# filaPro/unidet3d

Hardware: AMD Instinct MI355X
Metric: scenes/sec fwd+bwd, 100k-pt ScanNet voxel grid, 1/2/4/8 MI355X (higher is better)
Workload: dtype f32

## Files before the change

### unidet3d_amd/csrc/bn.hip

```cpp
#include <stdlib.h>

#include "u3d_common.h"

namespace u3d {

struct BnFin {
    double* sums;
    double rows;
    int set_rows;
    const float* gamma;
    const float* beta;
    float eps, momentum;
    float* running_mean;
    float* running_var;
    float* st;
    int64_t* nbt;
};

__device__ __forceinline__ void bn_finalize_channel(double s1, double s2, double rows, const float* gamma, const float* beta, float eps,
                                                    float momentum, float* running_mean, float* running_var, float* mean, float* invstd,
                                                    float* scale, float* shift, int c) {
#pragma clang fp contract(off)
    const double m = s1 / rows;
    double var = fma(-m, m, s2 / rows);
    if (var < 0.0) var = 0.0;
    const float is = (float)(1.0 / sqrt(var + (double)eps));
    const float mf = (float)m;
    mean[c] = mf;
    invstd[c] = is;
    const float sc = gamma[c] * is;
    scale[c] = sc;
    shift[c] = fmaf(-mf, sc, beta[c]);
    if (running_mean) {
        const double unbiased = rows > 1.0 ? var * rows / (rows - 1.0) : var;
        const float keep = 1.f - momentum;
        const float km = keep * running_mean[c], kv = keep * running_var[c];
        const float nm = momentum * mf, nv = momentum * (float)unbiased;
        running_mean[c] = km + nm;
        running_var[c] = kv + nv;
    }
}

__device__ __forceinline__ void bn_finish_body(const double* partial, int nblk, int C, const BnFin& f, int wave0, int nw, bool first) {
    const int lane = threadIdx.x & 63;
    for (int c = wave0; c < C; c += nw) {
        double t1 = 0.0, t2 = 0.0;
        for (int b = lane; b < nblk; b += 64) {
            t1 += partial[(int64_t)b * 2 * C + c];
            t2 += partial[(int64_t)b * 2 * C + C + c];
        }
#pragma unroll
        for (int d = 32; d >= 1; d >>= 1) { t1 += __shfl_xor(t1, d, 64); t2 += __shfl_xor(t2, d, 64); }
        if (lane) continue;
        f.sums[c] = t1;
        f.sums[C + c] = t2;
        if (!f.st) continue;
        bn_finalize_channel(t1, t2, f.rows, f.gamma, f.beta, f.eps, f.momentum, f.running_mean, f.running_var, f.st, f.st + C,
                            f.st + 2 * C, f.st + 3 * C, c);
    }
    if (first && threadIdx.x == 0) {
        if (f.set_rows) f.sums[2 * C] = f.rows;
        if (f.nbt) *f.nbt += 1;
    }
}

__global__ __launch_bounds__(256) void bn_sum_k(const double* __restrict__ partial, int nblk, int C, BnFin f) {
    bn_finish_body(partial, nblk, C, f, blockIdx.x * 4 + (threadIdx.x >> 6), gridDim.x * 4, blockIdx.x == 0);
}

template <int MODE>
__global__ __launch_bounds__(256) void bn_reduce_k(const float* __restrict__ x, const float* __restrict__ dy,
                                                   const float* __restrict__ mean, const float* __restrict__ invstd,
                                                   const float* __restrict__ scale, const float* __restrict__ shift, int relu,
                                                   int64_t n, int C, double* sums ) {
    __shared__ double sh[256 * 8];
    const int lpr = C >> 2;
    const int rpb = 256 / lpr;
    const int tid = threadIdx.x;
    const int c4 = tid % lpr, slot = tid / lpr;
    double a[4] = {0, 0, 0, 0}, b[4] = {0, 0, 0, 0};
    if (slot < rpb) {
        float4 mu = make_float4(0, 0, 0, 0), is = mu, sc = mu, sf = mu;
        if (MODE == 1) {
            mu = *reinterpret_cast<const float4*>(mean + c4 * 4);
            is = *reinterpret_cast<const float4*>(invstd + c4 * 4);
            sc = *reinterpret_cast<const float4*>(scale + c4 * 4);
            sf = *reinterpret_cast<const float4*>(shift + c4 * 4);
        }
        const int64_t stride = (int64_t)gridDim.x * rpb;
        for (int64_t r0 = (int64_t)blockIdx.x * rpb + slot; r0 < n; r0 += 4 * stride) {
            float4 v4[4], g4[4];
#pragma unroll
            for (int u = 0; u < 4; ++u) {
                const int64_t r = r0 + u * stride;
                v4[u] = make_float4(0.f, 0.f, 0.f, 0.f);
                g4[u] = make_float4(0.f, 0.f, 0.f, 0.f);
                if (r < n) {
                    v4[u] = *reinterpret_cast<const float4*>(x + r * C + c4 * 4);
                    if (MODE == 1) g4[u] = *reinterpret_cast<const float4*>(dy + r * C + c4 * 4);
                }
            }
#pragma unroll
            for (int u = 0; u < 4; ++u) {
                const float4 v = v4[u];
                if (MODE == 0) {
                    a[0] += v.x; a[1] += v.y; a[2] += v.z; a[3] += v.w;
                    b[0] += (double)v.x * v.x; b[1] += (double)v.y * v.y; b[2] += (double)v.z * v.z; b[3] += (double)v.w * v.w;
                } else {
                    float4 g = g4[u];
                    if (relu) {
                        if (!(v.x * sc.x + sf.x > 0.f)) g.x = 0.f;
                        if (!(v.y * sc.y + sf.y > 0.f)) g.y = 0.f;
                        if (!(v.z * sc.z + sf.z > 0.f)) g.z = 0.f;
                        if (!(v.w * sc.w + sf.w > 0.f)) g.w = 0.f;
                    }
                    a[0] += g.x; a[1] += g.y; a[2] += g.z; a[3] += g.w;
                    b[0] += (double)g.x * ((v.x - mu.x) * is.x); b[1] += (double)g.y * ((v.y - mu.y) * is.y);
                    b[2] += (double)g.z * ((v.z - mu.z) * is.z); b[3] += (double)g.w * ((v.w - mu.w) * is.w);
                }
            }
        }
    }
#pragma unroll
    for (int j = 0; j < 4; ++j) { sh[tid * 8 + j] = a[j]; sh[tid * 8 + 4 + j] = b[j]; }
    __syncthreads();
    if (tid < lpr) {
        double ta[4] = {0, 0, 0, 0}, tb[4] = {0, 0, 0, 0};
        for (int s = 0; s < rpb; ++s) {
            const int o = (s * lpr + tid) * 8;
#pragma unroll
            for (int j = 0; j < 4; ++j) { ta[j] += sh[o + j]; tb[j] += sh[o + 4 + j]; }
        }
        double* out = sums + (int64_t)blockIdx.x * 2 * C;
#pragma unroll
        for (int j = 0; j < 4; ++j) {
            out[tid * 4 + j] = ta[j];
            out[C + tid * 4 + j] = tb[j];
        }
    }
}

__global__ __launch_bounds__(256) void bn_partials_k(const float* __restrict__ partial, int64_t n_tiles, int C, double* ws) {
    __shared__ double sh[256];
    const int C2 = 2 * C, tid = threadIdx.x;
    double* out = ws + (int64_t)blockIdx.x * C2;
    for (int c0 = 0; c0 < C2; c0 += 256) {
        const int w = min(256, C2 - c0), rpp = 256 / w;
        const int col = c0 + tid % w, slot = tid / w;
        double a0 = 0.0, a1 = 0.0;
        if (slot < rpp) {
            const int64_t step = (int64_t)gridDim.x * rpp;
            int64_t r = (int64_t)blockIdx.x * rpp + slot;
            for (; r + step < n_tiles; r += 2 * step) {
                a0 += (double)partial[r * C2 + col];
                a1 += (double)partial[(r + step) * C2 + col];
            }
            if (r < n_tiles) a0 += (double)partial[r * C2 + col];
        }
        sh[tid] = a0 + a1;
        __syncthreads();
        if (tid < w) {
            double t = 0.0;
            for (int s_ = 0; s_ < rpp; ++s_) t += sh[s_ * w + tid];
            out[c0 + tid] = t;
        }
        __syncthreads();
    }
}


__global__ void bn_finalize_k(const double* __restrict__ sums, double count, const float* __restrict__ gamma,
                              const float* __restrict__ beta, float eps, float momentum, float* running_mean,
                              float* running_var, int C, float* mean, float* invstd, float* scale, float* shift,
                              int64_t* num_batches_tracked) {
    const int c = blockIdx.x * blockDim.x + threadIdx.x;
    if (c == 0 && num_batches_tracked) *num_batches_tracked += 1;
    if (c >= C) return;
    if (!(count > 0.0)) count = sums[2 * C];
    bn_finalize_channel(sums[c], sums[C + c], count, gamma, beta, eps, momentum, running_mean, running_var, mean, invstd, scale, shift, c);
}


__global__ __launch_bounds__(256) void bn_apply_k(const float* __restrict__ x, const float* __restrict__ scale,
                                                  const float* __restrict__ shift, int relu, int64_t n4, int C4, float* y, __bf16* yb) {
    for (int64_t i = (int64_t)blockIdx.x * blockDim.x + threadIdx.x; i < n4; i += (int64_t)gridDim.x * blockDim.x) {
        const int c4 = (int)(i % C4);
        const float4 v = reinterpret_cast<const float4*>(x)[i];
        const float4 sc = reinterpret_cast<const float4*>(scale)[c4];
        const float4 sf = reinterpret_cast<const float4*>(shift)[c4];
        const float4 o = bn_affine_relu(v, sc, sf, relu);
        reinterpret_cast<float4*>(y)[i] = o;
        if (yb) store_shadow(yb, i / C4, C4, 0, c4, o);
    }
}

__global__ __launch_bounds__(256) void bn_bwd_apply_k(const float* __restrict__ x, const float* __restrict__ dy,
                                                      const float* __restrict__ mean, const float* __restrict__ invstd,
                                                      const float* __restrict__ scale, const float* __restrict__ shift, int relu,
                                                      const double* __restrict__ sums, double inv_count, int64_t n4, int C,
                                                      float* dx, float* dgamma, float* dbeta, const double* __restrict__ count_src,
                                                      const float* __restrict__ addend, __bf16* dxb) {
    const int C4 = C >> 2;
    if (!(inv_count > 0.0)) inv_count = 1.0 / (count_src ? count_src[0] : sums[2 * C]);
    if (blockIdx.x == 0 && dgamma) {
        for (int c = threadIdx.x; c < C; c += blockDim.x) {
            dbeta[c] = (float)sums[c];
            dgamma[c] = (float)sums[C + c];
        }
    }
    for (int64_t i = (int64_t)blockIdx.x * blockDim.x + threadIdx.x; i < n4; i += (int64_t)gridDim.x * blockDim.x) {
        const int c4 = (int)(i % C4);
        const float4 v = reinterpret_cast<const float4*>(x)[i];
        float4 g = reinterpret_cast<const float4*>(dy)[i];
        const float4 mu = reinterpret_cast<const float4*>(mean)[c4];
        const float4 is = reinterpret_cast<const float4*>(invstd)[c4];
        const float4 sc = reinterpret_cast<const float4*>(scale)[c4];
        const float4 sf = reinterpret_cast<const float4*>(shift)[c4];
        if (relu) {
            if (!(v.x * sc.x + sf.x > 0.f)) g.x = 0.f;
            if (!(v.y * sc.y + sf.y > 0.f)) g.y = 0.f;
            if (!(v.z * sc.z + sf.z > 0.f)) g.z = 0.f;
            if (!(v.w * sc.w + sf.w > 0.f)) g.w = 0.f;
        }
        const int c = c4 * 4;
        const float m1x = (float)(sums[c] * inv_count), m1y = (float)(sums[c + 1] * inv_count);
        const float m1z = (float)(sums[c + 2] * inv_count), m1w = (float)(sums[c + 3] * inv_count);
        const float m2x = (float)(sums[C + c] * inv_count), m2y = (float)(sums[C + c + 1] * inv_count);
        const float m2z = (float)(sums[C + c + 2] * inv_count), m2w = (float)(sums[C + c + 3] * inv_count);
        float4 o;
        o.x = sc.x * (g.x - m1x - (v.x - mu.x) * is.x * m2x);
        o.y = sc.y * (g.y - m1y - (v.y - mu.y) * is.y * m2y);
        o.z = sc.z * (g.z - m1z - (v.z - mu.z) * is.z * m2z);
        o.w = sc.w * (g.w - m1w - (v.w - mu.w) * is.w * m2w);
        if (addend) {
            const float4 e = reinterpret_cast<const float4*>(addend)[i];
            o.x += e.x; o.y += e.y; o.z += e.z; o.w += e.w;
        }
        reinterpret_cast<float4*>(dx)[i] = o;
        if (dxb) store_shadow(dxb, i / C4, C4, 0, c4, o);
    }
}

static bool bn_ok(int64_t n, int C) { return n > 0 && C >= 4 && C <= 512 && C % 4 == 0; }
static bool shadow_ok(const void* sh, int C) { return !sh || C % 32 == 0; }
static unsigned ew_grid(int64_t n4) {
    int64_t g = ceil_div(n4, 256);
    return (unsigned)(g < 1 ? 1 : (g > 4096 ? 4096 : g));
}

}

using namespace u3d;

extern "C" {

static int bn_grid(int64_t n, int C) {
    const int rpb = 256 / (C / 4);
    int64_t g = ceil_div(n, (int64_t)rpb * 16);
    return (int)(g < 1 ? 1 : (g > 256 ? 256 : g));
}
static int bn_partials_grid(int64_t n_tiles, int C) {
    const int rpp = 2 * C >= 256 ? 1 : 256 / (2 * C);
    int64_t g = ceil_div(n_tiles, (int64_t)rpp * 16);
    return (int)(g < 1 ? 1 : (g > 128 ? 128 : g));
}

int64_t u3d_bn_ws_bytes(int C) { return (int64_t)256 * 2 * C * sizeof(double) + 64; }

static int bn_finish_launch(const void* ws, int nblk, int C, const BnFin& f, hipStream_t s) {
    hipLaunchKernelGGL(bn_sum_k, dim3((C + 3) / 4), dim3(256), 0, s, (const double*)ws, nblk, C, f);
    return check_launch("bn_sum");
}

static BnFin bn_fin(double* sums, double rows, int set_rows) {
    BnFin f;
    f.sums = sums; f.rows = rows; f.set_rows = set_rows; f.gamma = nullptr; f.beta = nullptr; f.eps = 0.f; f.momentum = 0.f;
    f.running_mean = nullptr; f.running_var = nullptr; f.st = nullptr; f.nbt = nullptr;
    return f;
}

static int bn_stats_launch(const float* x, int64_t n, int C, const float* partial, int64_t n_tiles, const BnFin& f, void* ws, hipStream_t s) {
    if (partial) {
        if (n_tiles <= 0) return U3D_EINVAL;
        ProfScope prof(U3D_K_BN, s, (double)n_tiles * C * 8);
        const int g = bn_partials_grid(n_tiles, C);
        hipLaunchKernelGGL(bn_partials_k, dim3(g), dim3(256), 0, s, partial, n_tiles, C, (double*)ws);
        return bn_finish_launch(ws, g, C, f, s);
    }
    ProfScope prof(U3D_K_BN, s, (double)n * C * 4);
    const int g = bn_grid(n, C);
    hipLaunchKernelGGL(bn_reduce_k<0>, dim3(g), dim3(256), 0, s, x, (const float*)nullptr, (const float*)nullptr,
                       (const float*)nullptr, (const float*)nullptr, (const float*)nullptr, 0, n, C, (double*)ws);
    return bn_finish_launch(ws, g, C, f, s);
}

int u3d_bn_stats(const float* x, int64_t n, int C, const float* partial, int64_t n_tiles, double* sums, void* ws, u3d_stream_t stream) {
    if ((!x && !partial) || !sums || !ws || !bn_ok(n, C)) return U3D_EINVAL;
    return bn_stats_launch(x, n, C, partial, n_tiles, bn_fin(sums, (double)n, 1), ws, (hipStream_t)stream);
}

int u3d_bn_finalize(const double* sums, double count, const float* gamma, const float* beta, float eps, float momentum,
                    float* running_mean, float* running_var, int C, float* mean, float* invstd, float* scale,
                    float* shift, int64_t* num_batches_tracked, u3d_stream_t stream) {
    if (!sums || !gamma || !beta || !mean || !invstd || !scale || !shift || C <= 0) return U3D_EINVAL;
    hipLaunchKernelGGL(bn_finalize_k, dim3((C + 63) / 64), dim3(64), 0, (hipStream_t)stream, sums, count, gamma, beta, eps,
                       momentum, running_mean, running_var, C, mean, invstd, scale, shift, num_batches_tracked);
    return check_launch("bn_finalize");
}

int u3d_bn_apply(const float* x, const float* scale, const float* shift, int relu, int64_t n, int C, float* y, void* y_bf16,
                 u3d_stream_t stream) {
    if (!x || !scale || !shift || !y || !bn_ok(n, C) || !shadow_ok(y_bf16, C)) return U3D_EINVAL;
    hipStream_t s = (hipStream_t)stream;
    ProfScope prof(U3D_K_BN, s, (double)n * C * (y_bf16 ? 10 : 8));
    const int64_t n4 = n * (C / 4);
    hipLaunchKernelGGL(bn_apply_k, dim3(ew_grid(n4)), dim3(256), 0, s, x, scale, shift, relu, n4, C / 4, y, (__bf16*)y_bf16);
    return check_launch("bn_apply");
}

int u3d_bn_bwd_stats(const float* x, const float* dy, const float* mean, const float* invstd, const float* scale,
                     const float* shift, int relu, int64_t n, int C, double* sums, void* ws, u3d_stream_t stream) {
    if (!x || !dy || !mean || !invstd || !scale || !shift || !sums || !ws || !bn_ok(n, C)) return U3D_EINVAL;
    hipStream_t s = (hipStream_t)stream;
    ProfScope prof(U3D_K_BN, s, (double)n * C * 8);
    const int g = bn_grid(n, C);
    const BnFin f = bn_fin(sums, 0.0, 0);
    hipLaunchKernelGGL(bn_reduce_k<1>, dim3(g), dim3(256), 0, s, x, dy, mean, invstd, scale, shift, relu, n, C, (double*)ws);
    return bn_finish_launch(ws, g, C, f, s);
}

int u3d_bn_bwd_apply(const float* x, const float* dy, const float* mean, const float* invstd, const float* scale,
                     const float* shift, int relu, const double* sums, double count, int64_t n, int C, float* dx, void* dx_bf16,
                     float* dgamma, float* dbeta, const float* addend, u3d_stream_t stream) {
    if (!x || !dy || !mean || !invstd || !scale || !shift || !sums || !dx || !bn_ok(n, C) || !shadow_ok(dx_bf16, C)) return U3D_EINVAL;
    hipStream_t s = (hipStream_t)stream;
    ProfScope prof(U3D_K_BN, s, (double)n * C * 12);
    const int64_t n4 = n * (C / 4);
    hipLaunchKernelGGL(bn_bwd_apply_k, dim3(ew_grid(n4)), dim3(256), 0, s, x, dy, mean, invstd, scale, shift, relu, sums,
                       1.0 / count, n4, C, dx, dgamma, dbeta, (const double*)nullptr, addend, (__bf16*)dx_bf16);
    return check_launch("bn_bwd_apply");
}

int u3d_bn_forward(const float* x, int64_t n, int C, const float* partial, int64_t n_tiles, const float* gamma, const float* beta, float eps,
                   float momentum, float* running_mean, float* running_var, int64_t* num_batches_tracked, int relu, float* y, void* y_bf16,
                   float* st, double* sums, void* ws, u3d_stream_t stream) {
    if (!x || !sums || !ws || !gamma || !beta || !st || !y || !bn_ok(n, C) || !shadow_ok(y_bf16, C)) return U3D_EINVAL;
    if (partial && n_tiles <= 0) return U3D_EINVAL;
    BnFin f = bn_fin(sums, (double)n, 1);
    f.gamma = gamma; f.beta = beta; f.eps = eps; f.momentum = momentum; f.running_mean = running_mean; f.running_var = running_var;
    f.st = st; f.nbt = num_batches_tracked;
    int rc = bn_stats_launch(x, n, C, partial, n_tiles, f, ws, (hipStream_t)stream);
    if (rc) return rc;
    return u3d_bn_apply(x, st + 2 * C, st + 3 * C, relu, n, C, y, y_bf16, stream);
}

int u3d_bn_backward(const float* x, const float* dy, const float* st, int relu, const double* fwd_sums, double* sums, int64_t n, int C,
                    float* dx, void* dx_bf16, float* dgamma, float* dbeta, const float* addend, void* ws, u3d_stream_t stream) {
    if (!fwd_sums || !st || !dx || !shadow_ok(dx_bf16, C)) return U3D_EINVAL;
    int rc = u3d_bn_bwd_stats(x, dy, st, st + C, st + 2 * C, st + 3 * C, relu, n, C, sums, ws, stream);
    if (rc) return rc;
    hipStream_t s = (hipStream_t)stream;
    ProfScope prof(U3D_K_BN, s, (double)n * C * 12);
    const int64_t n4 = n * (C / 4);
    hipLaunchKernelGGL(bn_bwd_apply_k, dim3(ew_grid(n4)), dim3(256), 0, s, x, dy, (const float*)st, (const float*)(st + C), (const float*)(st + 2 * C),
                       (const float*)(st + 3 * C), relu, (const double*)sums, -1.0, n4, C, dx, dgamma, dbeta, fwd_sums + 2 * C, addend,
                       (__bf16*)dx_bf16);
    return check_launch("bn_backward");
}

}
```

Measured before the change: 310.9.

## Add single-kernel slab BatchNorm paths for small inputs and hoist per-channel constants

```diff
diff --git a/unidet3d_amd/csrc/bn.hip b/unidet3d_amd/csrc/bn.hip
--- a/unidet3d_amd/csrc/bn.hip
+++ b/unidet3d_amd/csrc/bn.hip
@@ -68,7 +68,7 @@
     bn_finish_body(partial, nblk, C, f, blockIdx.x * 4 + (threadIdx.x >> 6), gridDim.x * 4, blockIdx.x == 0);
 }
 
-template <int MODE>
+template <int MODE, int TRIP>
 __global__ __launch_bounds__(256) void bn_reduce_k(const float* __restrict__ x, const float* __restrict__ dy,
                                                    const float* __restrict__ mean, const float* __restrict__ invstd,
                                                    const float* __restrict__ scale, const float* __restrict__ shift, int relu,
@@ -88,10 +88,10 @@
             sf = *reinterpret_cast<const float4*>(shift + c4 * 4);
         }
         const int64_t stride = (int64_t)gridDim.x * rpb;
-        for (int64_t r0 = (int64_t)blockIdx.x * rpb + slot; r0 < n; r0 += 4 * stride) {
-            float4 v4[4], g4[4];
-#pragma unroll
-            for (int u = 0; u < 4; ++u) {
+        for (int64_t r0 = (int64_t)blockIdx.x * rpb + slot; r0 < n; r0 += TRIP * stride) {
+            float4 v4[TRIP], g4[TRIP];
+#pragma unroll
+            for (int u = 0; u < TRIP; ++u) {
                 const int64_t r = r0 + u * stride;
                 v4[u] = make_float4(0.f, 0.f, 0.f, 0.f);
                 g4[u] = make_float4(0.f, 0.f, 0.f, 0.f);
@@ -101,7 +101,7 @@
                 }
             }
 #pragma unroll
-            for (int u = 0; u < 4; ++u) {
+            for (int u = 0; u < TRIP; ++u) {
                 const float4 v = v4[u];
                 if (MODE == 0) {
                     a[0] += v.x; a[1] += v.y; a[2] += v.z; a[3] += v.w;
@@ -183,15 +183,36 @@
 
 __global__ __launch_bounds__(256) void bn_apply_k(const float* __restrict__ x, const float* __restrict__ scale,
                                                   const float* __restrict__ shift, int relu, int64_t n4, int C4, float* y, __bf16* yb) {
-    for (int64_t i = (int64_t)blockIdx.x * blockDim.x + threadIdx.x; i < n4; i += (int64_t)gridDim.x * blockDim.x) {
-        const int c4 = (int)(i % C4);
+    const int64_t i0 = (int64_t)blockIdx.x * blockDim.x + threadIdx.x;
+    const int c4 = (int)(i0 % C4);
+    const float4 sc = reinterpret_cast<const float4*>(scale)[c4];
+    const float4 sf = reinterpret_cast<const float4*>(shift)[c4];
+    for (int64_t i = i0; i < n4; i += (int64_t)gridDim.x * blockDim.x) {
         const float4 v = reinterpret_cast<const float4*>(x)[i];
-        const float4 sc = reinterpret_cast<const float4*>(scale)[c4];
-        const float4 sf = reinterpret_cast<const float4*>(shift)[c4];
         const float4 o = bn_affine_relu(v, sc, sf, relu);
         reinterpret_cast<float4*>(y)[i] = o;
         if (yb) store_shadow(yb, i / C4, C4, 0, c4, o);
     }
+}
+
+struct BnBwdConst { float4 mu, is, sc, sf, m1, m2; };
+__device__ __forceinline__ float4 bn_bwd_elem(const float4& v, float4 g, const BnBwdConst& k, int relu, const float4* addend) {
+    if (relu) {
+        if (!(v.x * k.sc.x + k.sf.x > 0.f)) g.x = 0.f;
+        if (!(v.y * k.sc.y + k.sf.y > 0.f)) g.y = 0.f;
+        if (!(v.z * k.sc.z + k.sf.z > 0.f)) g.z = 0.f;
+        if (!(v.w * k.sc.w + k.sf.w > 0.f)) g.w = 0.f;
+    }
+    float4 o;
+    o.x = k.sc.x * (g.x - k.m1.x - (v.x - k.mu.x) * k.is.x * k.m2.x);
+    o.y = k.sc.y * (g.y - k.m1.y - (v.y - k.mu.y) * k.is.y * k.m2.y);
+    o.z = k.sc.z * (g.z - k.m1.z - (v.z - k.mu.z) * k.is.z * k.m2.z);
+    o.w = k.sc.w * (g.w - k.m1.w - (v.w - k.mu.w) * k.is.w * k.m2.w);
+    if (addend) {
+        const float4 e = *addend;
+        o.x += e.x; o.y += e.y; o.z += e.z; o.w += e.w;
+    }
+    return o;
 }
 
 __global__ __launch_bounds__(256) void bn_bwd_apply_k(const float* __restrict__ x, const float* __restrict__ dy,
@@ -208,44 +229,226 @@
             dgamma[c] = (float)sums[C + c];
         }
     }
-    for (int64_t i = (int64_t)blockIdx.x * blockDim.x + threadIdx.x; i < n4; i += (int64_t)gridDim.x * blockDim.x) {
-        const int c4 = (int)(i % C4);
+    const int64_t i0 = (int64_t)blockIdx.x * blockDim.x + threadIdx.x;
+    const int c4 = (int)(i0 % C4);
+    const int c = c4 * 4;
+    BnBwdConst k;
+    k.mu = reinterpret_cast<const float4*>(mean)[c4];
+    k.is = reinterpret_cast<const float4*>(invstd)[c4];
+    k.sc = reinterpret_cast<const float4*>(scale)[c4];
+    k.sf = reinterpret_cast<const float4*>(shift)[c4];
+    k.m1 = make_float4((float)(sums[c] * inv_count), (float)(sums[c + 1] * inv_count), (float)(sums[c + 2] * inv_count), (float)(sums[c + 3] * inv_count));
+    k.m2 = make_float4((float)(sums[C + c] * inv_count), (float)(sums[C + c + 1] * inv_count), (float)(sums[C + c + 2] * inv_count),
+                       (float)(sums[C + c + 3] * inv_count));
+    for (int64_t i = i0; i < n4; i += (int64_t)gridDim.x * blockDim.x) {
         const float4 v = reinterpret_cast<const float4*>(x)[i];
-        float4 g = reinterpret_cast<const float4*>(dy)[i];
-        const float4 mu = reinterpret_cast<const float4*>(mean)[c4];
-        const float4 is = reinterpret_cast<const float4*>(invstd)[c4];
-        const float4 sc = reinterpret_cast<const float4*>(scale)[c4];
-        const float4 sf = reinterpret_cast<const float4*>(shift)[c4];
-        if (relu) {
-            if (!(v.x * sc.x + sf.x > 0.f)) g.x = 0.f;
-            if (!(v.y * sc.y + sf.y > 0.f)) g.y = 0.f;
-            if (!(v.z * sc.z + sf.z > 0.f)) g.z = 0.f;
-            if (!(v.w * sc.w + sf.w > 0.f)) g.w = 0.f;
-        }
-        const int c = c4 * 4;
-        const float m1x = (float)(sums[c] * inv_count), m1y = (float)(sums[c + 1] * inv_count);
-        const float m1z = (float)(sums[c + 2] * inv_count), m1w = (float)(sums[c + 3] * inv_count);
-        const float m2x = (float)(sums[C + c] * inv_count), m2y = (float)(sums[C + c + 1] * inv_count);
-        const float m2z = (float)(sums[C + c + 2] * inv_count), m2w = (float)(sums[C + c + 3] * inv_count);
-        float4 o;
-        o.x = sc.x * (g.x - m1x - (v.x - mu.x) * is.x * m2x);
-        o.y = sc.y * (g.y - m1y - (v.y - mu.y) * is.y * m2y);
-        o.z = sc.z * (g.z - m1z - (v.z - mu.z) * is.z * m2z);
-        o.w = sc.w * (g.w - m1w - (v.w - mu.w) * is.w * m2w);
-        if (addend) {
-            const float4 e = reinterpret_cast<const float4*>(addend)[i];
-            o.x += e.x; o.y += e.y; o.z += e.z; o.w += e.w;
-        }
+        const float4 g = reinterpret_cast<const float4*>(dy)[i];
+        const float4 o = bn_bwd_elem(v, g, k, relu, addend ? reinterpret_cast<const float4*>(addend) + i : nullptr);
         reinterpret_cast<float4*>(dx)[i] = o;
         if (dxb) store_shadow(dxb, i / C4, C4, 0, c4, o);
     }
 }
 
+#define BN_SLAB_THREADS 1024
+#define BN_SLAB_WAVES (BN_SLAB_THREADS / 64)
+
+__device__ __forceinline__ void bn_slab_sum(const double* a, const double* b, double* sh) {
+    const int tid = threadIdx.x;
+    double v[8];
+#pragma unroll
+    for (int j = 0; j < 4; ++j) { v[j] = a[j]; v[4 + j] = b[j]; }
+#pragma unroll
+    for (int j = 0; j < 8; ++j) {
+#pragma unroll
+        for (int d = 32; d >= 1; d >>= 1) v[j] += __shfl_xor(v[j], d, 64);
+    }
+    if ((tid & 63) == 0) {
+#pragma unroll
+        for (int j = 0; j < 8; ++j) sh[(tid >> 6) * 8 + j] = v[j];
+    }
+    __syncthreads();
+    if (tid < 8) {
+        double t = 0.0;
+        for (int w = 0; w < BN_SLAB_WAVES; ++w) t += sh[w * 8 + tid];
+        sh[8 * BN_SLAB_WAVES + tid] = t;
+    }
+    __syncthreads();
+}
+
+__global__ __launch_bounds__(BN_SLAB_THREADS) void bn_slab_fwd_k(const float* __restrict__ x, int64_t n, int C, BnFin f, int relu, float* y, __bf16* yb) {
+    __shared__ double sh[8 * BN_SLAB_WAVES + 8];
+    __shared__ float cst[8];
+    const int C4 = C >> 2, c4 = blockIdx.x, tid = threadIdx.x;
+    const float4* xc = reinterpret_cast<const float4*>(x) + c4;
+    double a[4] = {0, 0, 0, 0}, b[4] = {0, 0, 0, 0};
+    for (int64_t r0 = tid; r0 < n; r0 += 4 * BN_SLAB_THREADS) {
+        float4 v4[4];
+#pragma unroll
+        for (int u = 0; u < 4; ++u) {
+            const int64_t r = r0 + u * BN_SLAB_THREADS;
+            v4[u] = r < n ? xc[r * C4] : make_float4(0.f, 0.f, 0.f, 0.f);
+        }
+#pragma unroll
+        for (int u = 0; u < 4; ++u) {
+            const float4 v = v4[u];
+            a[0] += v.x; a[1] += v.y; a[2] += v.z; a[3] += v.w;
+            b[0] += (double)v.x * v.x; b[1] += (double)v.y * v.y; b[2] += (double)v.z * v.z; b[3] += (double)v.w * v.w;
+        }
+    }
+    bn_slab_sum(a, b, sh);
+    if (tid < 4) {
+        const int c = c4 * 4 + tid;
+        const double t1 = sh[8 * BN_SLAB_WAVES + tid], t2 = sh[8 * BN_SLAB_WAVES + 4 + tid];
+        f.sums[c] = t1;
+        f.sums[C + c] = t2;
+        if (f.st) {
+            bn_finalize_channel(t1, t2, f.rows, f.gamma, f.beta, f.eps, f.momentum, f.running_mean, f.running_var, f.st, f.st + C, f.st + 2 * C,
+                                f.st + 3 * C, c);
+            cst[tid] = f.st[2 * C + c];
+            cst[4 + tid] = f.st[3 * C + c];
+        }
+    }
+    if (c4 == 0 && tid == 0) {
+        if (f.set_rows) f.sums[2 * C] = f.rows;
+        if (f.nbt) *f.nbt += 1;
+    }
+    if (!y) return;
+    __syncthreads();
+    const float4 sc = make_float4(cst[0], cst[1], cst[2], cst[3]), sf = make_float4(cst[4], cst[5], cst[6], cst[7]);
+    for (int64_t r = tid; r < n; r += BN_SLAB_THREADS) {
+        const float4 v = xc[r * C4];
+        const float4 o = bn_affine_relu(v, sc, sf, relu);
+        reinterpret_cast<float4*>(y)[r * C4 + c4] = o;
+        if (yb) store_shadow(yb, r, C4, 0, c4, o);
+    }
+}
+
+__global__ __launch_bounds__(BN_SLAB_THREADS) void bn_slab_bwd_k(const float* __restrict__ x, const float* __restrict__ dy,
+                                                                 const float* __restrict__ mean, const float* __restrict__ invstd,
+                                                                 const float* __restrict__ scale, const float* __restrict__ shift, int relu,
+                                                                 int64_t n, int C, double* sums, const double* __restrict__ count_src, float* dx,
+                                                                 float* dgamma, float* dbeta, const float* __restrict__ addend, __bf16* dxb) {
+    __shared__ double sh[8 * BN_SLAB_WAVES + 8];
+    const int C4 = C >> 2, c4 = blockIdx.x, tid = threadIdx.x;
+    const float4* xc = reinterpret_cast<const float4*>(x) + c4;
+    const float4* gc = reinterpret_cast<const float4*>(dy) + c4;
+    BnBwdConst k;
+    k.mu = reinterpret_cast<const float4*>(mean)[c4];
+    k.is = reinterpret_cast<const float4*>(invstd)[c4];
+    k.sc = reinterpret_cast<const float4*>(scale)[c4];
+    k.sf = reinterpret_cast<const float4*>(shift)[c4];
+    const float4 mu = k.mu, is = k.is, sc = k.sc, sf = k.sf;
+    double a[4] = {0, 0, 0, 0}, b[4] = {0, 0, 0, 0};
+    for (int64_t r0 = tid; r0 < n; r0 += 4 * BN_SLAB_THREADS) {
+        float4 v4[4], g4[4];
+#pragma unroll
+        for (int u = 0; u < 4; ++u) {
+            const int64_t r = r0 + u * BN_SLAB_THREADS;
+            v4[u] = make_float4(0.f, 0.f, 0.f, 0.f);
+            g4[u] = make_float4(0.f, 0.f, 0.f, 0.f);
+            if (r < n) { v4[u] = xc[r * C4]; g4[u] = gc[r * C4]; }
+        }
+#pragma unroll
+        for (int u = 0; u < 4; ++u) {
+            const float4 v = v4[u];
+            float4 g = g4[u];
+            if (relu) {
+                if (!(v.x * sc.x + sf.x > 0.f)) g.x = 0.f;
+                if (!(v.y * sc.y + sf.y > 0.f)) g.y = 0.f;
+                if (!(v.z * sc.z + sf.z > 0.f)) g.z = 0.f;
+                if (!(v.w * sc.w + sf.w > 0.f)) g.w = 0.f;
+            }
+            a[0] += g.x; a[1] += g.y; a[2] += g.z; a[3] += g.w;
+            b[0] += (double)g.x * ((v.x - mu.x) * is.x); b[1] += (double)g.y * ((v.y - mu.y) * is.y);
+            b[2] += (double)g.z * ((v.z - mu.z) * is.z); b[3] += (double)g.w * ((v.w - mu.w) * is.w);
+        }
+    }
+    bn_slab_sum(a, b, sh);
+    const double* tot = sh + 8 * BN_SLAB_WAVES;
+    if (tid < 4) {
+        const int c = c4 * 4 + tid;
+        sums[c] = tot[tid];
+        sums[C + c] = tot[4 + tid];
+        if (dx && dgamma) {
+            dbeta[c] = (float)tot[tid];
+            dgamma[c] = (float)tot[4 + tid];
+        }
+    }
+    if (!dx) return;
+    const double inv_count = 1.0 / count_src[0];
+    k.m1 = make_float4((float)(tot[0] * inv_count), (float)(tot[1] * inv_count), (float)(tot[2] * inv_count), (float)(tot[3] * inv_count));
+    k.m2 = make_float4((float)(tot[4] * inv_count), (float)(tot[5] * inv_count), (float)(tot[6] * inv_count), (float)(tot[7] * inv_count));
+    for (int64_t r = tid; r < n; r += BN_SLAB_THREADS) {
+        const int64_t i = r * C4 + c4;
+        const float4 o = bn_bwd_elem(xc[r * C4], gc[r * C4], k, relu, addend ? reinterpret_cast<const float4*>(addend) + i : nullptr);
+        reinterpret_cast<float4*>(dx)[i] = o;
+        if (dxb) store_shadow(dxb, r, C4, 0, c4, o);
+    }
+}
+
 static bool bn_ok(int64_t n, int C) { return n > 0 && C >= 4 && C <= 512 && C % 4 == 0; }
 static bool shadow_ok(const void* sh, int C) { return !sh || C % 32 == 0; }
-static unsigned ew_grid(int64_t n4) {
+static unsigned apply_grid(int64_t n4, int C4) {
     int64_t g = ceil_div(n4, 256);
-    return (unsigned)(g < 1 ? 1 : (g > 4096 ? 4096 : g));
+    g = g < 1 ? 1 : (g > 4096 ? 4096 : g);
+    int a = C4, b = 256;
+    while (b) { const int t = a % b; a = b; b = t; }
+    const int m = C4 / a;
+    return (unsigned)(ceil_div(g, m) * m);
+}
+
+#if defined(U3D_BN_CAP) && U3D_BN_CAP > 512
+#define BN_MAX_GRID U3D_BN_CAP
+#else
+#define BN_MAX_GRID 512
+#endif
+static const int64_t BN_STREAM_BYTES = (int64_t)8 << 20;
+struct BnPlan { int grid, trip; };
+static BnPlan bn_plan(int mode, int64_t n, int C) {
+    const int rpb = 256 / (C / 4);
+    int cap = 256, trip = 4;
+    if (mode == 0 && n * C * 4 >= BN_STREAM_BYTES) cap = 512;
+#ifdef U3D_BN_CAP
+    cap = U3D_BN_CAP;
+#endif
+#ifdef U3D_BN_TRIP
+    trip = U3D_BN_TRIP;
+#endif
+    int64_t g = ceil_div(n, (int64_t)rpb * 16);
+    BnPlan p;
+    p.grid = (int)(g < 1 ? 1 : (g > cap ? cap : g));
+    p.trip = trip;
+    return p;
+}
+template <int MODE>
+static void bn_reduce_launch(const BnPlan& p, hipStream_t s, const float* x, const float* dy, const float* mean, const float* invstd,
+                             const float* scale, const float* shift, int relu, int64_t n, int C, double* ws) {
+    if (p.trip == 8)
+        hipLaunchKernelGGL((bn_reduce_k<MODE, 8>), dim3(p.grid), dim3(256), 0, s, x, dy, mean, invstd, scale, shift, relu, n, C, ws);
+    else
+        hipLaunchKernelGGL((bn_reduce_k<MODE, 4>), dim3(p.grid), dim3(256), 0, s, x, dy, mean, invstd, scale, shift, relu, n, C, ws);
+}
+
+static bool bn_slab(int mode, int64_t n) {
+#ifdef U3D_BN_SLAB_ROWS
+    return n <= U3D_BN_SLAB_ROWS;
+#else
+    return n <= (mode == 0 ? 2000 : 815);
+#endif
+}
+
+static int bn_slab_fwd_launch(const float* x, int64_t n, int C, const BnFin& f, int relu, float* y, void* y_bf16, hipStream_t s) {
+    ProfScope prof(U3D_K_BN, s, (double)n * C * (y ? (y_bf16 ? 14 : 12) : 4));
+    hipLaunchKernelGGL(bn_slab_fwd_k, dim3(C / 4), dim3(BN_SLAB_THREADS), 0, s, x, n, C, f, relu, y, (__bf16*)y_bf16);
+    return check_launch("bn_slab_fwd");
+}
+static int bn_slab_bwd_launch(const float* x, const float* dy, const float* mean, const float* invstd, const float* scale, const float* shift,
+                              int relu, int64_t n, int C, double* sums, const double* count_src, float* dx, void* dx_bf16, float* dgamma,
+                              float* dbeta, const float* addend, hipStream_t s) {
+    ProfScope prof(U3D_K_BN, s, (double)n * C * (dx ? 20 : 8));
+    hipLaunchKernelGGL(bn_slab_bwd_k, dim3(C / 4), dim3(BN_SLAB_THREADS), 0, s, x, dy, mean, invstd, scale, shift, relu, n, C, sums, count_src, dx,
+                       dgamma, dbeta, addend, (__bf16*)dx_bf16);
+    return check_launch("bn_slab_bwd");
 }
 
 }
@@ -254,18 +457,13 @@
 
 extern "C" {
 
-static int bn_grid(int64_t n, int C) {
-    const int rpb = 256 / (C / 4);
-    int64_t g = ceil_div(n, (int64_t)rpb * 16);
-    return (int)(g < 1 ? 1 : (g > 256 ? 256 : g));
-}
 static int bn_partials_grid(int64_t n_tiles, int C) {
     const int rpp = 2 * C >= 256 ? 1 : 256 / (2 * C);
     int64_t g = ceil_div(n_tiles, (int64_t)rpp * 16);
     return (int)(g < 1 ? 1 : (g > 128 ? 128 : g));
 }
 
-int64_t u3d_bn_ws_bytes(int C) { return (int64_t)256 * 2 * C * sizeof(double) + 64; }
+int64_t u3d_bn_ws_bytes(int C) { return (int64_t)BN_MAX_GRID * 2 * C * sizeof(double) + 64; }
 
 static int bn_finish_launch(const void* ws, int nblk, int C, const BnFin& f, hipStream_t s) {
     hipLaunchKernelGGL(bn_sum_k, dim3((C + 3) / 4), dim3(256), 0, s, (const double*)ws, nblk, C, f);
@@ -287,11 +485,11 @@
         hipLaunchKernelGGL(bn_partials_k, dim3(g), dim3(256), 0, s, partial, n_tiles, C, (double*)ws);
         return bn_finish_launch(ws, g, C, f, s);
     }
+    if (bn_slab(0, n)) return bn_slab_fwd_launch(x, n, C, f, 0, nullptr, nullptr, s);
     ProfScope prof(U3D_K_BN, s, (double)n * C * 4);
-    const int g = bn_grid(n, C);
-    hipLaunchKernelGGL(bn_reduce_k<0>, dim3(g), dim3(256), 0, s, x, (const float*)nullptr, (const float*)nullptr,
-                       (const float*)nullptr, (const float*)nullptr, (const float*)nullptr, 0, n, C, (double*)ws);
-    return bn_finish_launch(ws, g, C, f, s);
+    const BnPlan p = bn_plan(0, n, C);
+    bn_reduce_launch<0>(p, s, x, nullptr, nullptr, nullptr, nullptr, nullptr, 0, n, C, (double*)ws);
+    return bn_finish_launch(ws, p.grid, C, f, s);
 }
 
 int u3d_bn_stats(const float* x, int64_t n, int C, const float* partial, int64_t n_tiles, double* sums, void* ws, u3d_stream_t stream) {
@@ -314,7 +512,7 @@
     hipStream_t s = (hipStream_t)stream;
     ProfScope prof(U3D_K_BN, s, (double)n * C * (y_bf16 ? 10 : 8));
     const int64_t n4 = n * (C / 4);
-    hipLaunchKernelGGL(bn_apply_k, dim3(ew_grid(n4)), dim3(256), 0, s, x, scale, shift, relu, n4, C / 4, y, (__bf16*)y_bf16);
+    hipLaunchKernelGGL(bn_apply_k, dim3(apply_grid(n4, C / 4)), dim3(256), 0, s, x, scale, shift, relu, n4, C / 4, y, (__bf16*)y_bf16);
     return check_launch("bn_apply");
 }
 
@@ -322,11 +520,13 @@
                      const float* shift, int relu, int64_t n, int C, double* sums, void* ws, u3d_stream_t stream) {
     if (!x || !dy || !mean || !invstd || !scale || !shift || !sums || !ws || !bn_ok(n, C)) return U3D_EINVAL;
     hipStream_t s = (hipStream_t)stream;
+    if (bn_slab(1, n))
+        return bn_slab_bwd_launch(x, dy, mean, invstd, scale, shift, relu, n, C, sums, nullptr, nullptr, nullptr, nullptr, nullptr, nullptr, s);
     ProfScope prof(U3D_K_BN, s, (double)n * C * 8);
-    const int g = bn_grid(n, C);
+    const BnPlan p = bn_plan(1, n, C);
     const BnFin f = bn_fin(sums, 0.0, 0);
-    hipLaunchKernelGGL(bn_reduce_k<1>, dim3(g), dim3(256), 0, s, x, dy, mean, invstd, scale, shift, relu, n, C, (double*)ws);
-    return bn_finish_launch(ws, g, C, f, s);
+    bn_reduce_launch<1>(p, s, x, dy, mean, invstd, scale, shift, relu, n, C, (double*)ws);
+    return bn_finish_launch(ws, p.grid, C, f, s);
 }
 
 int u3d_bn_bwd_apply(const float* x, const float* dy, const float* mean, const float* invstd, const float* scale,
@@ -336,7 +536,7 @@
     hipStream_t s = (hipStream_t)stream;
     ProfScope prof(U3D_K_BN, s, (double)n * C * 12);
     const int64_t n4 = n * (C / 4);
-    hipLaunchKernelGGL(bn_bwd_apply_k, dim3(ew_grid(n4)), dim3(256), 0, s, x, dy, mean, invstd, scale, shift, relu, sums,
+    hipLaunchKernelGGL(bn_bwd_apply_k, dim3(apply_grid(n4, C / 4)), dim3(256), 0, s, x, dy, mean, invstd, scale, shift, relu, sums,
                        1.0 / count, n4, C, dx, dgamma, dbeta, (const double*)nullptr, addend, (__bf16*)dx_bf16);
     return check_launch("bn_bwd_apply");
 }
@@ -349,6 +549,7 @@
     BnFin f = bn_fin(sums, (double)n, 1);
     f.gamma = gamma; f.beta = beta; f.eps = eps; f.momentum = momentum; f.running_mean = running_mean; f.running_var = running_var;
     f.st = st; f.nbt = num_batches_tracked;
+    if (!partial && bn_slab(0, n)) return bn_slab_fwd_launch(x, n, C, f, relu, y, y_bf16, (hipStream_t)stream);
     int rc = bn_stats_launch(x, n, C, partial, n_tiles, f, ws, (hipStream_t)stream);
     if (rc) return rc;
     return u3d_bn_apply(x, st + 2 * C, st + 3 * C, relu, n, C, y, y_bf16, stream);
@@ -357,12 +558,16 @@
 int u3d_bn_backward(const float* x, const float* dy, const float* st, int relu, const double* fwd_sums, double* sums, int64_t n, int C,
                     float* dx, void* dx_bf16, float* dgamma, float* dbeta, const float* addend, void* ws, u3d_stream_t stream) {
     if (!fwd_sums || !st || !dx || !shadow_ok(dx_bf16, C)) return U3D_EINVAL;
+    if (!x || !dy || !sums || !ws || !bn_ok(n, C)) return U3D_EINVAL;
+    if (bn_slab(1, n))
+        return bn_slab_bwd_launch(x, dy, st, st + C, st + 2 * C, st + 3 * C, relu, n, C, sums, fwd_sums + 2 * C, dx, dx_bf16, dgamma, dbeta, addend,
+                                  (hipStream_t)stream);
     int rc = u3d_bn_bwd_stats(x, dy, st, st + C, st + 2 * C, st + 3 * C, relu, n, C, sums, ws, stream);
     if (rc) return rc;
     hipStream_t s = (hipStream_t)stream;
     ProfScope prof(U3D_K_BN, s, (double)n * C * 12);
     const int64_t n4 = n * (C / 4);
-    hipLaunchKernelGGL(bn_bwd_apply_k, dim3(ew_grid(n4)), dim3(256), 0, s, x, dy, (const float*)st, (const float*)(st + C), (const float*)(st + 2 * C),
+    hipLaunchKernelGGL(bn_bwd_apply_k, dim3(apply_grid(n4, C / 4)), dim3(256), 0, s, x, dy, (const float*)st, (const float*)(st + C), (const float*)(st + 2 * C),
                        (const float*)(st + 3 * C), relu, (const double*)sums, -1.0, n4, C, dx, dgamma, dbeta, fwd_sums + 2 * C, addend,
                        (__bf16*)dx_bf16);
     return check_launch("bn_backward");
```

After: 312.6, median of 6. Within noise of the previous version (+0.5%).
